# rajashree-srikanth/drone-sim-python

Hardware: AMD Instinct MI355X
Metric: trajectory-optimisations/sec (6-seg poly, 50 wpts) (higher is better)
Workload: dtype f64 residual/gradient + f32 MFMA J^T J

## Files before the change

### drone-sim-python_amd/csrc/asan_host.cpp

```cpp
#include <cmath>
#include <cstdarg>
#include <cstdio>
#include <string>

#include "fit_plan.h"

static std::string g_err;
void d2d_set_error(const char *fmt, ...) {
  char buf[512];
  va_list ap;
  va_start(ap, fmt);
  vsnprintf(buf, sizeof(buf), fmt, ap);
  va_end(ap);
  g_err = buf;
}

static int check_plan(int S, int K, double duration) {
  d2d_fit_plan pl;
  pl.device = 0; pl.S = S; pl.K = K; pl.duration = duration;
  const double s = 0.1 / K;
  pl.wref[0] = 4e-4; pl.wref[1] = 5.0 * s; pl.wref[2] = s / (9.81 * 9.81);
  const int rc = fit_basis_build(&pl);
  if (rc != 0) { std::printf("S=%d K=%d: rc=%d (%s)\n", S, K, rc, g_err.c_str()); return rc; }
  const int nq = pl.nq;
  double worst = 0.0;
  for (int i = 0; i < nq; ++i)
    for (int j = 0; j < nq; ++j) {
      double acc = 0.0;
      for (int k = 0; k < K; ++k) acc += pl.Pinit[(size_t)i * K + k] * pl.G[(size_t)k * nq + j];
      worst = std::fmax(worst, std::fabs(acc - (i == j ? 1.0 : 0.0)));
    }
  std::printf("S=%d K=%d nq=%d: |Pinit G0 - I| = %.2e\n", S, K, nq, worst);
  if (int rc2 = fit_basis_segments(&pl)) { std::printf("  segments: rc=%d (%s)\n", rc2, g_err.c_str()); return rc2; }
  double wseg = 0.0, gmax = 0.0;
  const double c1 = 2.0 / pl.T;
  for (int k = 0; k < K; ++k) {
    const double x = pl.sx[k];
    double P[8], d1[8], d2[8];
    P[0] = 1; P[1] = x; d1[0] = 0; d1[1] = 1; d2[0] = d2[1] = 0;
    for (int n = 1; n < 7; ++n) {
      P[n + 1] = ((2.0 * n + 1.0) * x * P[n] - n * P[n - 1]) / (n + 1.0);
      d1[n + 1] = d1[n - 1] + (2.0 * n + 1.0) * P[n];
      d2[n + 1] = d2[n - 1] + (2.0 * n + 1.0) * d1[n];
    }
    for (int d = 0; d < 3; ++d)
      for (int j = 0; j < nq; ++j) {
        double acc = 0.0;
        for (int i = 0; i < 8; ++i) {
          const double psi = d == 0 ? P[i] : (d == 1 ? c1 * d1[i] : c1 * c1 * d2[i]);
          acc += psi * pl.Zl[(size_t)(8 * pl.seg[k] + i) * nq + j];
        }
        const double gv = pl.G[((size_t)d * K + k) * nq + j];
        wseg = std::fmax(wseg, std::fabs(acc - gv));
        gmax = std::fmax(gmax, std::fabs(gv));
      }
  }
  int lanes = 0, covered = 0, zlbig = 0;
  for (int s = 0; s < S; ++s) {
    const int L = pl.seg_l0[s + 1] - pl.seg_l0[s];
    lanes += L;
    covered += pl.seg_Ks[s];
    if (L < 1 || (pl.seg_Ks[s] + L - 1) / L > pl.seg_nchunk) zlbig = 1;
  }
  double zlmax = 0.0;
  for (double v : pl.Zl) zlmax = std::fmax(zlmax, std::fabs(v));
  std::printf("  segments: |Psi Zl - G| = %.2e of %.2e, |Zl| <= %.2f, %d lanes, %d chunks\n", wseg, gmax, zlmax, lanes, pl.seg_nchunk);
  if (!(wseg < 1e-9 * gmax) || lanes > 64 || covered != K || zlbig || !(zlmax < 50.0)) return 1;
  return worst < 1e-6 ? 0 : 1;
}

int main() {
  int bad = 0;
  const int shapes[][2] = {{6, 50}, {6, 61}, {6, 121}, {6, 151}, {6, 501}, {3, 20}, {1, 8}, {4, 31}};
  for (auto &sh : shapes) bad += check_plan(sh[0], sh[1], 0.1 * (sh[1] - 1)) != 0;
  d2d_fit_plan pl;
  pl.device = 0; pl.S = 6; pl.K = 18; pl.duration = 1.0; pl.wref[0] = 4e-4; pl.wref[1] = 1e-2; pl.wref[2] = 1e-5;
  const int rc = fit_basis_build(&pl);
  std::printf("S=6 K=18 (rank-deficient): rc=%d (%s)\n", rc, g_err.c_str());
  bad += rc == 0;
  std::printf(bad ? "asan_host: FAILED\n" : "asan_host: ok\n");
  return bad;
}
```

### drone-sim-python_amd/csrc/fit_basis.cpp

```cpp
#include <cmath>
#include <cstring>

#include "fit_plan.h"

namespace {

double arr(int k, int n) {
  double a = 1;
  for (int i = n; i > n - k; --i) a *= i;
  return a;
}

struct Dense {
  int r, c;
  std::vector<double> a;
  Dense(int r_, int c_) : r(r_), c(c_), a((size_t)r_ * c_, 0.0) {}
  double &operator()(int i, int j) { return a[(size_t)i * c + j]; }
  double operator()(int i, int j) const { return a[(size_t)i * c + j]; }
};

Dense matmul(const Dense &A, const Dense &B, bool tA = false) {
  const int m = tA ? A.c : A.r, k = tA ? A.r : A.c, n = B.c;
  Dense C(m, n);
  for (int i = 0; i < m; ++i)
    for (int l = 0; l < k; ++l) {
      const double v = tA ? A(l, i) : A(i, l);
      if (v == 0.0) continue;
      for (int j = 0; j < n; ++j) C(i, j) += v * B(l, j);
    }
  return C;
}

bool cholesky(Dense &A) {
  const int n = A.r;
  for (int j = 0; j < n; ++j) {
    double d = A(j, j);
    for (int k = 0; k < j; ++k) d -= A(j, k) * A(j, k);
    if (!(d > 0.0)) return false;
    d = std::sqrt(d);
    A(j, j) = d;
    for (int i = j + 1; i < n; ++i) {
      double s = A(i, j);
      for (int k = 0; k < j; ++k) s -= A(i, k) * A(j, k);
      A(i, j) = s / d;
    }
    for (int i = 0; i < j; ++i) A(i, j) = 0.0;
  }
  return true;
}

bool invert(Dense &A) {
  const int n = A.r;
  Dense I(n, n);
// ... 229 lines not shown
          (best < 0 || chunks(s) > chunks(best) || (chunks(s) == chunks(best) && pl->seg_Ks[s] * L[best] > pl->seg_Ks[best] * L[s])))
        best = s;
    if (best < 0) break;
    L[best]++;
  }
  pl->seg_nchunk = 0;
  pl->seg_l0[0] = 0;
  for (int s = 0; s < S; ++s) {
    pl->seg_l0[s + 1] = pl->seg_l0[s] + L[s];
    if (chunks(s) > pl->seg_nchunk) pl->seg_nchunk = chunks(s);
  }
  for (int s = S; s < D2D_FIT_MAX_S; ++s) pl->seg_l0[s + 1] = pl->seg_l0[S];
  return D2D_OK;
}

int fit_basis_knots(d2d_fit_plan *pl) {
  const int S = pl->S, K = pl->K, nq = pl->nq, NE = 8 * (S + 1);
  const double T = pl->T;
  if (nq != 4 * S || (int)pl->Lw.size() != nq * nq) { d2d_set_error("fit_basis_knots: plan without the whitening factor"); return D2D_EINVAL; }
  auto &kn = pl->kn;
  kn.NE = NE;
  double dsc[4] = {1.0, T, T * T / 2.0, T * T * T / 6.0};
  std::vector<int> freec;
  for (int i = 0; i < 4 * (S + 1); ++i)
    if (i != 0 && i != 1 && i != 4 * S && i != 4 * S + 1) freec.push_back(i);
  const int NV = 4 * (S + 1);
  kn.NV = NV;
  std::vector<int> vfree(NV, -1);
  for (int i = 0; i < nq; ++i) vfree[freec[i]] = i;
  Dense A(8, 8);
  for (int k = 0; k < 4; ++k) {
    A(k, k) = 1.0;
    for (int p = k; p < 8; ++p) {
      double c = 1.0;
      for (int i = 0; i < k; ++i) c = c * (p - i) / (i + 1);
      A(4 + k, p) = c;
    }
  }
  if (!invert(A)) { d2d_set_error("fit_basis_knots: singular Hermite block"); return D2D_EINVAL; }
  kn.Hb64.assign((size_t)K * KN_HB_STRIDE, 0.0);
  kn.Hb32.assign((size_t)K * 32, 0.f);
  for (int k = 0; k < K; ++k) {
    const double x = pl->tau[k] / T;
    const int s = pl->seg[k];
    for (int d = 0; d < 3; ++d)
      for (int m = 0; m < 8; ++m) {
        double v = 0.0;
        for (int p = d; p < 8; ++p) v += arr(d, p) * std::pow(x, p - d) * A(p, m);
        v /= std::pow(T, d);
        kn.Hb64[(size_t)k * KN_HB_STRIDE + 4 * m + d] = v;
        const bool fixed = (s == 0 && m < 2) || (s == S - 1 && m >= 4 && m < 6);
        kn.Hb32[(size_t)k * 32 + 4 * m + d] = fixed ? 0.f : (float)v;
      }
  }
  fit_knot_first_samples(pl->seg, S, kn.k0);
  kn.Wseg.assign((size_t)S * 4 * 64, 0.f);
  for (int s = 0; s < S; ++s)
    for (int r = 0; r < 4; ++r)
      for (int l = 0; l < 64; ++l) {
        const int R = 4 * (l >> 4) + r, C = l & 15;
        const int aR = (R >> 2) & 1, aC = (C >> 2) & 1, mR = 4 * (R >> 3) + (R & 3), mC = 4 * (C >> 3) + (C & 3);
        if (aR != aC) continue;
        double v = 0.0;
        for (int k = kn.k0[s]; k < kn.k0[s + 1]; ++k) v += (double)kn.Hb32[(size_t)k * 32 + 4 * mR] * (double)kn.Hb32[(size_t)k * 32 + 4 * mC];
        kn.Wseg[((size_t)s * 4 + r) * 64 + l] = (float)v;
      }
  Dense L(nq, nq), Bm(nq, nq), Bi(nq, nq), Mu(nq, nq);
  for (int i = 0; i < nq; ++i)
    for (int j = 0; j < nq; ++j) L(i, j) = pl->Lw[(size_t)i * nq + j];
  std::vector<double> ds(nq);
  for (int i = 0; i < nq; ++i) ds[i] = dsc[freec[i] % 4];
  for (int j = 0; j < nq; ++j)
    for (int i = 0; i < nq; ++i) Bm(j, i) = L(i, j) / ds[i];
  Bi = Bm;
  if (!invert(Bi)) { d2d_set_error("fit_basis_knots: singular map"); return D2D_EINVAL; }
  Mu = matmul(Bm, Bm, true);
  Dense Mi = Mu;
  if (!invert(Mi)) { d2d_set_error("fit_basis_knots: singular metric"); return D2D_EINVAL; }
  kn.Bq.assign((size_t)2 * nq * NV, 0.0);
  kn.BiT.assign((size_t)2 * nq * NV, 0.0);
  kn.Md32.assign((size_t)2 * nq * 2 * nq, 0.f);
  kn.Mrow32.assign((size_t)NE * 12, 0.f);
  kn.Binv.assign((size_t)NE * nq, 0.0);
  kn.Minv.assign((size_t)NE * NV, 0.0);
  kn.Mrow.assign((size_t)NE * 12, 0.0);
  kn.Pu.assign((size_t)NE * 4, 0.0);
  kn.msc.assign((size_t)NE, 1.0);
  for (int a = 0; a < 2; ++a)
    for (int jq = 0; jq < nq; ++jq)
      for (int i = 0; i < nq; ++i) {
        kn.Bq[((size_t)a * nq + jq) * NV + freec[i]] = Bm(jq, i);
        kn.BiT[((size_t)a * nq + jq) * NV + freec[i]] = Bi(i, jq);
      }
  for (int e = 0; e < NE; ++e) {
    const int j = e >> 3, k = e & 3, v = 4 * j + k, i = vfree[v];
    if (i < 0) {
      kn.Pu[(size_t)e * 4 + (j == 0 ? k : 2 + k)] = dsc[k];
      continue;
    }
    for (int c = 0; c < 4; ++c) kn.Pu[(size_t)e * 4 + c] = ds[i] * pl->Pe[(size_t)i * 4 + c];
    for (int jq = 0; jq < nq; ++jq) kn.Binv[(size_t)e * nq + jq] = Bi(i, jq);
    for (int i2 = 0; i2 < nq; ++i2) kn.Minv[(size_t)e * NV + freec[i2]] = Mi(i, i2);
    for (int dj = -1; dj <= 1; ++dj)
      for (int k2 = 0; k2 < 4; ++k2) {
        const int v2 = 4 * (j + dj) + k2;
        if (v2 < 0 || v2 >= NV || vfree[v2] < 0) continue;
// ... 24 lines not shown
```

### drone-sim-python_amd/csrc/fit_knot.hip

```cpp
#include <cstdlib>
#include <vector>

#include "fit_phases.h"
#include "fit_plan.h"

#define KN_WPB_MAX 8
#define KN_LDS_BYTES (160 * 1024)
#define KN_N 48
#define KN_NE 56
#define KN_WV_KNOT 10
#define KN_US 10
#define KN_GTOL_SCALE 0.1
#define KN_SEG_MAX 11
#define KN_FUSED_DEPTH 6
#define KN_SEG_FLOOR 8
#define KN_IMG_LS (KN_N + 4)

namespace {

#define LAUNDER_S(v) do { (v) = __builtin_amdgcn_readfirstlane(v); asm volatile("" : "+s"(v)); } while (0)

struct KnotGeom {
  int K, S, smax;
  int k0[D2D_FIT_MAX_S + 2];
// ... 126 lines not shown
          h01[i] = *reinterpret_cast<const f64x2a *>(hb + i * KN_HB_STRIDE); u01[i] = *reinterpret_cast<const f64x2a *>(uk + i * KN_US);
          h2[i] = hb[i * KN_HB_STRIDE + 2]; u2[i] = uk[i * KN_US + 2];
        } else {
          h01[i] = f64x2a{0.0, 0.0}; u01[i] = f64x2a{0.0, 0.0}; h2[i] = 0.0; u2[i] = 0.0;
        }
#pragma unroll
      for (int i = 0; i < 3; ++i) {
        a0 = fma(h01[i].x, u01[i].x, a0);
        a1 = fma(h01[i].y, u01[i].y, a1);
        a2 = fma(h2[i], u2[i], a2);
      }
      hb += 3 * KN_HB_STRIDE; uk += 3 * KN_US;
    }
  }
  return (a0 + a1) + a2;
}

template <int SEGMAX>
__device__ __forceinline__ void knot_mfma(const KnotGeom &kg, const unsigned char *lds, int hb32_off, int cf_off, const float *Wseg,
                                          float ww, int lane, f32x4 (&acc)[D2D_FIT_MAX_S]) {
  LAUNDER(lane);
  const int c = lane & 15, r = lane >> 4;
  const int m = 4 * (c >> 3) + (c & 3), a = (c >> 2) & 1;
  const int tab = hb32_off + (4 * m + (r < 2 ? 1 : 0)) * 4;
  const int cfo = cf_off + r * 16 + a * 8;
#pragma unroll
  for (int s0 = 0; s0 < D2D_FIT_MAX_S; s0 += 3) {
    float v[3][SEGMAX];
    int n[3];
#pragma unroll
    for (int j = 0; j < 3; ++j) {
      const int s = s0 + j;
      int kb = kg.k0[s];
      n[j] = kg.k0[s + 1] - kg.k0[s];
      LAUNDER_S(kb); LAUNDER_S(n[j]);
#pragma unroll
      for (int i = 0; i < SEGMAX; ++i) {
        const int kk = kb + (i < n[j] ? i : (n[j] > 0 ? n[j] - 1 : 0));
        const float2 t = lds_get<float2>(lds + tab + kk * 128);
        const float2 cc = lds_get<float2>(lds + cfo + kk * 64);
        v[j][i] = fmaf(cc.y, t.y, cc.x * t.x);
      }
#pragma unroll
      for (int rr = 0; rr < 4; ++rr) acc[s][rr] = ww * Wseg[(s * 4 + rr) * 64 + lane];
    }
#pragma unroll
    for (int i = 0; i < SEGMAX; ++i)
#pragma unroll
      for (int j = 0; j < 3; ++j)
        if (i < n[j]) acc[s0 + j] = __builtin_amdgcn_mfma_f32_16x16x4f32(v[j][i], v[j][i], acc[s0 + j], 0, 0, 0);
  }
}

template <int SEGMAX, int SEGMIN>
__device__ __forceinline__ double knot_eval_fused(const KnotGeom &kg, const unsigned char *lds, const double *Hb64, const double *us,
                                                  int kb, int km, int ke, int a, int kd, bool live, int hb32_off, int cf_off,
                                                  const float *Wseg, float ww, int lane, f32x4 (&acc)[D2D_FIT_MAX_S]) {
  typedef double __attribute__((ext_vector_type(2), may_alias)) f64x2a;
  constexpr int SLOTS = (SEGMAX + 2) / 3 * 3;
  static_assert(SEGMIN > 0 && SEGMIN <= SEGMAX && SEGMIN % 3 != 0, "a masked sample follows the floor in every half");
  static_assert(D2D_FIT_MAX_S == 6, "two halves of three segments");
  LAUNDER(lane);
  LAUNDER(kb);
  const int c = lane & 15, r = lane >> 4;
  const int m = 4 * (c >> 3) + (c & 3), ax = (c >> 2) & 1;
  const int tab = hb32_off + (4 * m + (r < 2 ? 1 : 0)) * 4;
  const int cfo = cf_off + r * 16 + ax * 8;
  double a0 = 0.0, a1 = 0.0, a2 = 0.0;
#pragma unroll
  for (int half = 0; half < 2; ++half) {
    const int s0 = 3 * half;
    const int k0 = half ? km : kb, k1 = half ? ke : km;
    const int n = live ? k1 - k0 : 0;
    const bool some = n > 0;
    const int k0r = some ? k0 : 0;
    const double *hb = Hb64 + (size_t)k0r * KN_HB_STRIDE + 4 * ((half ? 0 : 4) + kd);
    const double *uk = us + k0r * KN_US + 4 * a;
    const double b0 = a0, b1 = a1, b2 = a2;
    constexpr int NQ = 3 * SEGMIN, TAIL = SEGMAX - SEGMIN, DEPTH = KN_FUSED_DEPTH;
    static_assert(SEGMIN >= 4, "the operand pipeline is two rows deep");
    const unsigned char *tp[3], *cp[3];
    float2 rt[DEPTH], rc[DEPTH], rtt[3][TAIL > 0 ? TAIL : 1], rct[3][TAIL > 0 ? TAIL : 1];
    float vq[2], vt[3][TAIL > 0 ? TAIL : 1];
    int ns[3];
#pragma unroll
    for (int j = 0; j < 3; ++j) {
      const int s = s0 + j;
      int sb = kg.k0[s];
      ns[j] = kg.k0[s + 1] - kg.k0[s];
      LAUNDER_S(sb); LAUNDER_S(ns[j]);
      tp[j] = lds + tab + sb * 128; cp[j] = lds + cfo + sb * 64;
#pragma unroll
      for (int i = 0; i < DEPTH / 3; ++i) { rt[3 * i + j] = lds_get<float2>(tp[j] + i * 128); rc[3 * i + j] = lds_get<float2>(cp[j] + i * 64); }
#pragma unroll
      for (int rr = 0; rr < 4; ++rr) acc[s][rr] = ww * Wseg[(s * 4 + rr) * 64 + lane];
    }
    vq[0] = fmaf(rc[0].y, rt[0].y, rc[0].x * rt[0].x);
    __builtin_amdgcn_sched_barrier(0);
    constexpr int LAG = 3, STEP = (NQ - 1 - LAG) / (SLOTS - 1), NBUF = LAG / (STEP > 0 ? STEP : 1) + 1;
    static_assert(STEP >= 1, "every sample of the half finds its two k-steps");
    f64x2a h01[NBUF], u01[NBUF];
    double h2[NBUF], u2[NBUF];
    auto p2_read = [&](int idx, int i) {
      if (idx < SEGMIN) {
        h01[i] = *reinterpret_cast<const f64x2a *>(hb + idx * KN_HB_STRIDE); u01[i] = *reinterpret_cast<const f64x2a *>(uk + idx * KN_US);
        h2[i] = hb[idx * KN_HB_STRIDE + 2]; u2[i] = uk[idx * KN_US + 2];
      } else {
        const bool in = idx < n;
        const int o = in ? idx : 0;
        const f64x2a hr = *reinterpret_cast<const f64x2a *>(hb + o * KN_HB_STRIDE), ur = *reinterpret_cast<const f64x2a *>(uk + o * KN_US);
        const double h2r = hb[o * KN_HB_STRIDE + 2], u2r = uk[o * KN_US + 2];
        h01[i] = in ? hr : f64x2a{0.0, 0.0}; u01[i] = in ? ur : f64x2a{0.0, 0.0};
        h2[i] = in ? h2r : 0.0; u2[i] = in ? u2r : 0.0;
      }
    };
    auto p2_fma = [&](int idx, int i) {
      if (idx == SEGMIN) { a0 = some ? a0 : b0; a1 = some ? a1 : b1; a2 = some ? a2 : b2; }
      a0 = fma(h01[i].x, u01[i].x, a0);
      a1 = fma(h01[i].y, u01[i].y, a1);
      a2 = fma(h2[i], u2[i], a2);
      LAUNDER(a0); LAUNDER(a1); LAUNDER(a2);
    };
#pragma unroll
    for (int q = 0; q < NQ; ++q) {
      const int i = q / 3, j = q % 3;
      acc[s0 + j] = __builtin_amdgcn_mfma_f32_16x16x4f32(vq[q & 1], vq[q & 1], acc[s0 + j], 0, 0, 0);
      if (q + DEPTH < NQ) {
        rt[q % DEPTH] = lds_get<float2>(tp[j] + (i + DEPTH / 3) * 128); rc[q % DEPTH] = lds_get<float2>(cp[j] + (i + DEPTH / 3) * 64);
      } else if (q + 6 < NQ + 3 && q + 6 >= NQ) {
#pragma unroll
        for (int t = 0; t < TAIL; ++t) {
          const int kk = SEGMIN + t < ns[j] ? SEGMIN + t : ns[j] - 1;
          rtt[j][t] = lds_get<float2>(tp[j] + kk * 128); rct[j][t] = lds_get<float2>(cp[j] + kk * 64);
        }
      } else if (q + 3 >= NQ) {
#pragma unroll
        for (int t = 0; t < TAIL; ++t) vt[j][t] = fmaf(rct[j][t].y, rtt[j][t].y, rct[j][t].x * rtt[j][t].x);
      }
      if (q % STEP == 0 && q / STEP < SLOTS) p2_read(q / STEP, (q / STEP) % NBUF);
      if (q >= LAG && (q - LAG) % STEP == 0 && (q - LAG) / STEP < SLOTS) p2_fma((q - LAG) / STEP, ((q - LAG) / STEP) % NBUF);
      if (q + 1 < NQ) vq[(q + 1) & 1] = fmaf(rc[(q + 1) % DEPTH].y, rt[(q + 1) % DEPTH].y, rc[(q + 1) % DEPTH].x * rt[(q + 1) % DEPTH].x);
      __builtin_amdgcn_sched_barrier(0);
    }
#pragma unroll
    for (int t = 0; t < TAIL; ++t)
#pragma unroll
      for (int j = 0; j < 3; ++j)
        if (SEGMIN + t < ns[j]) acc[s0 + j] = __builtin_amdgcn_mfma_f32_16x16x4f32(vt[j][t], vt[j][t], acc[s0 + j], 0, 0, 0);
  }
  return (a0 + a1) + a2;
}

__device__ __forceinline__ void knot_mfma_so(const KnotGeom &kg, const unsigned char *lds, int hb32_off, int cf_off, int cfp_off,
                                             const float *Wseg, float ww, int lane, f32x4 (&acc)[D2D_FIT_MAX_S]) {
  LAUNDER(lane);
  const int c = lane & 15, rho = lane >> 4;
  const int m = 4 * (c >> 3) + (c & 3);
  const bool ay = ((c >> 2) & 1) != 0, row_y = (rho & 1) != 0, row_2 = rho >= 2;
  const int tab = hb32_off + 4 * m * 4;
  const int reco = cf_off + rho * 16 + (ay ? 8 : 0), rpo = cfp_off + (rho & 1) * 8 + (ay ? 4 : 0);
#pragma unroll
  for (int s = 0; s < D2D_FIT_MAX_S; ++s) {
#pragma unroll
    for (int rr = 0; rr < 4; ++rr) acc[s][rr] = ww * Wseg[(s * 4 + rr) * 64 + lane];
    int k1 = kg.k0[s + 1];
    int k = kg.k0[s];
    LAUNDER_S(k1); LAUNDER_S(k);
    if (k < k1) {
      f32x4 hb = lds_get<f32x4>(lds + tab + k * 128);
      float2 rec = lds_get<float2>(lds + reco + k * 64);
      float rp = lds_get<float>(lds + rpo + k * 16);
      for (; k < k1; ++k) {
        const int kn = k + 1 < k1 ? k + 1 : k;
        const f32x4 hbn = lds_get<f32x4>(lds + tab + kn * 128);
        const float2 recn = lds_get<float2>(lds + reco + kn * 64);
        const float rpn = lds_get<float>(lds + rpo + kn * 16);
        const float h0 = hb.x, h1 = hb.y, h2 = hb.z;
        const float cx = rec.x, cy = rec.y;
        const float vb = fmaf(cy, h2, cx * h1);
        const float va = (row_y == ay) ? (row_2 ? h2 : h1) : 0.f;
        acc[s] = __builtin_amdgcn_mfma_f32_16x16x4f32(va, vb, acc[s], 0, 0, 0);
        const float vbp = row_2 ? 0.f : rp * h0;
        const float vap = (!row_2 && row_y == ay) ? h0 : 0.f;
        acc[s] = __builtin_amdgcn_mfma_f32_16x16x4f32(vap, vbp, acc[s], 0, 0, 0);
        hb = hbn; rec = recn; rp = rpn;
      }
    }
  }
}

__device__ __forceinline__ void knot_blocks_to_image(f32x4 (&acc)[D2D_FIT_MAX_S], float *Hs, int lane) {
  LAUNDER(lane);
  constexpr int LS = KN_IMG_LS;
  for (int i = lane; i < KN_N * LS / 4; i += 64) lds_put<f32x4>(Hs + 4 * i, f32x4{0.f, 0.f, 0.f, 0.f});
  const int c = lane & 15, g4 = lane >> 4;
  const bool lowq = c < 8 && g4 < 2, highq = c >= 8 && g4 >= 2;
  const int src = ((lane + 40) & 63) << 2;
  auto fetch = [&](float v) -> float {
    const float up = __builtin_bit_cast(float, __builtin_amdgcn_ds_bpermute(src, __builtin_bit_cast(int, v)));
    return lowq ? up : 0.f;
  };
#pragma unroll
  for (int s = D2D_FIT_MAX_S - 1; s >= 1; --s) {
    const float u0 = fetch(acc[s - 1].x), u1 = fetch(acc[s - 1].y), u2 = fetch(acc[s - 1].z), u3 = fetch(acc[s - 1].w);
    acc[s].x += u0; acc[s].y += u1; acc[s].z += u2; acc[s].w += u3;
  }
  wave_lds_sync();
  const int cq = c & 7, cd = 2 * (cq >> 2) + (cq & 3) - 2;
  const bool cv = (cq & 3) >= 2;
#pragma unroll
  for (int s = 0; s < D2D_FIT_MAX_S; ++s) {
    int iC = 8 * s + c - 4;
    bool okc = true;
    if (s == 0) { iC = c < 8 ? cd : c - 4; okc = c >= 8 || cv; }
    if (s == D2D_FIT_MAX_S - 1) { iC = c < 8 ? 8 * s + c - 4 : 44 + cd; okc = c < 8 || cv; }
    const bool mine = okc && !(highq && s < D2D_FIT_MAX_S - 1);
#pragma unroll
    for (int rr = 0; rr < 4; ++rr) {
      int iR = 8 * s + 4 * g4 + rr - 4;
      bool okr = true;
      if (s == 0 && rr < 2) okr = g4 >= 2;
      if (s == 0 && rr >= 2) iR = g4 < 2 ? 2 * g4 + rr - 2 : 4 * g4 + rr - 4;
      if (s == D2D_FIT_MAX_S - 1 && rr < 2) okr = g4 < 2;
      if (s == D2D_FIT_MAX_S - 1 && rr >= 2) iR = g4 < 2 ? 8 * s + 4 * g4 + rr - 4 : 44 + 2 * (g4 - 2) + rr - 2;
      if (mine && okr) Hs[iR * LS + iC] = acc[s][rr];
    }
  }
  wave_lds_sync();
}

struct KnotMetric {
  unsigned char *lds;
  int sfull_off, md32_off, mr32_off;
  int lane;
  float lam;
  float scale;
  __device__ __forceinline__ float apply(float v) const {
#ifdef KN_ABL_APPLY
    return v;
#endif
    int l = lane;
    LAUNDER(l);
    const bool act = l < KN_N;
    const int e = act ? kn_entry_of(l) : 0;
    float *sf = reinterpret_cast<float *>(lds + sfull_off);
    wave_lds_sync();
    if (act) sf[8 + e] = v;
    wave_lds_sync();
    const float *bq = sf + 8 * (e >> 3) + 4 * ((e >> 2) & 1);
    const float *mrow = reinterpret_cast<const float *>(lds + mr32_off) + e * 12;
    const f32x4 s0 = lds_get<f32x4>(bq), s1 = lds_get<f32x4>(bq + 8), s2 = lds_get<f32x4>(bq + 16);
    const f32x4 m0 = lds_get<f32x4>(mrow), m1 = lds_get<f32x4>(mrow + 4), m2 = lds_get<f32x4>(mrow + 8);
    float r = m0.x * s0.x;
    r = fmaf(m0.y, s0.y, r); r = fmaf(m0.z, s0.z, r); r = fmaf(m0.w, s0.w, r);
    r = fmaf(m1.x, s1.x, r); r = fmaf(m1.y, s1.y, r); r = fmaf(m1.z, s1.z, r); r = fmaf(m1.w, s1.w, r);
    r = fmaf(m2.x, s2.x, r); r = fmaf(m2.y, s2.y, r); r = fmaf(m2.z, s2.z, r); r = fmaf(m2.w, s2.w, r);
    return act ? r : 0.f;
  }
  int row_off;
  __device__ __forceinline__ void prepare(int l) { row_off = md32_off + ((l < KN_N && lam != 0.f) ? l : KN_N) * (KN_N * 4); }
  __device__ __forceinline__ f32x4 damp(int j0) const {
#ifdef KN_ABL_DAMP
    return f32x4{lam, lam, lam, lam};
#endif
    return lds_get<f32x4>(reinterpret_cast<const float *>(lds + row_off) + j0);
  }
};

}
template <> struct nd_is_banded<KnotMetric> { static constexpr bool value = true; };
static_assert(KN_N == 48 && D2D_FIT_MAX_S == 6, "nd_panel3_chunk0_zero<KnotMetric> rests on the 4 / 8 x 5 / 4 layout of the 48 free entries");
template <> struct nd_panel3_chunk0_zero<KnotMetric> { static constexpr bool value = true; };
namespace {

template <bool STAMPS, bool SEG9, int SEGMIN>
__global__ void __launch_bounds__(64 * KN_WPB_MAX)
fit_lm_knot_kernel(int B, KnotGeom kg, KnotLds L, d2d_fit_opts opts, int iter_cap, KnotDev T, const double *__restrict__ pk,
                   const double *__restrict__ prep, double *q_io, double *cost_io, double *g_io, double *lm, int32_t *flags,
                   int32_t *queue, const int32_t *__restrict__ order, int prio_at, double *u_io, unsigned long long *__restrict__ stamps,
                   float *dbg) {
  unsigned long long st_acc[8] = {0, 0, 0, 0, 0, 0, 0, 0}, st_last = 0;
#define KN_STAMP(i)                                                     \
  if (STAMPS) {                                                         \
    const unsigned long long t_ = __builtin_amdgcn_s_memtime();         \
    st_acc[i] += t_ - st_last;                                          \
    st_last = t_;                                                       \
  }
  extern __shared__ __attribute__((aligned(16))) unsigned char lds[];
  constexpr int N = KN_N;
  stage(lds + L.Hb64, T.Hb64, kg.K * KN_HB_STRIDE * 8);
  stage(lds + L.Hb32, T.Hb32, kg.K * 32 * 4);
  stage(lds + L.Wseg, T.Wseg, D2D_FIT_MAX_S * 4 * 64 * 4);
  stage(lds + L.Md32, T.Md32, N * N * 4);
  stage(lds + L.Mi32, T.Mi32, KN_NE * 28 * 4);
  stage(lds + L.Mr32, T.Mrow32, KN_NE * 12 * 4);
  stage(lds + L.Msc, T.msc, KN_NE * 8);
  for (int i = threadIdx.x; i < N; i += blockDim.x) reinterpret_cast<float *>(lds + L.Md32)[N * N + i] = 0.f;
  __syncthreads();
  const double *Hb64 = reinterpret_cast<const double *>(lds + L.Hb64);
  const float *Wseg = reinterpret_cast<const float *>(lds + L.Wseg);
  const float *Mi32 = reinterpret_cast<const float *>(lds + L.Mi32);
  const int wave = __builtin_amdgcn_readfirstlane(threadIdx.x >> 6), lane = threadIdx.x & 63;
  unsigned char *wl = lds + L.wave0 + wave * L.wave_stride;
  double *wv = reinterpret_cast<double *>(wl + L.wv);
  double *sp = reinterpret_cast<double *>(wl + L.sp);
  float *sfull = reinterpret_cast<float *>(wl + L.sfull);
  double *gfull = reinterpret_cast<double *>(wl + L.gfull);
  double *park = reinterpret_cast<double *>(wl + L.park);
  double *us = reinterpret_cast<double *>(wl + L.big);
  f32x4 *cf = reinterpret_cast<f32x4 *>(wl + L.cf);
  float2 *cfp = reinterpret_cast<float2 *>(wl + L.cfp);
  float *big = reinterpret_cast<float *>(wl + L.big);
  const bool act = lane < N;
  const int e = kn_entry_all(lane);
  const int ej = e >> 3, ea = (e >> 2) & 1, ekd = e & 3;
  const int wv_slot = ej * KN_WV_KNOT + 4 * ea + ekd;
  auto p2_ranges = [&](int &kb, int &km, int &ke) {
    int lj = lane;
    LAUNDER(lj);
    const int e2 = lj < N ? kn_entry_of(lj) : 0, j2 = e2 >> 3;
    kb = 0; km = 0; ke = 0;
#pragma unroll
    for (int j = 0; j <= D2D_FIT_MAX_S; ++j)
      if (j == j2) { kb = kg.k0[j > 0 ? j - 1 : 0]; km = kg.k0[j]; ke = kg.k0[j < kg.S ? j + 1 : kg.S]; }
  };
  auto seg_of_lane = [&]() -> int {
    int lj = lane;
    LAUNDER(lj);
    int sg = 0;
#pragma unroll
    for (int s = 1; s < D2D_FIT_MAX_S; ++s) sg += (lj >= kg.k0[s] && s < kg.S) ? 1 : 0;
    return sg;
  };
  auto msc_of_lane = [&]() -> double {
    int l = lane;
    LAUNDER(l);
    return reinterpret_cast<const double *>(lds + L.Msc)[l < N ? kn_entry_of(l) : 0];
  };
  for (int i = lane; i < 9 * 8; i += 64) sfull[i] = 0.f;
  KnotMetric metric;
  metric.lds = lds; metric.sfull_off = L.wave0 + wave * L.wave_stride + L.sfull; metric.md32_off = L.Md32; metric.mr32_off = L.Mr32;
  metric.lane = lane; metric.lam = 0.f; metric.scale = 0.f; metric.row_off = 0;
// ... 81 lines not shown
#define V_qmax u2
#define V_ct u3
#define V_pred_s u4
#define V_bt_a u5
#define V_bt_b u6
#define V_alpha u7
    int nev = 0, status = D2D_ST_RUNNING;
    bool so_rows = uniform_i(lmb[3] != 0.0 ? 1 : 0) != 0;
    int phase = 1;
    MpState mp;
    mp.pgn_lds = nullptr;
    mp.dx_gn = 0.0; mp.t2_gn = 0.0; mp.p_gn = 0.f; mp.gn_valid = 0; mp.gn_ok = 0; mp.first = 0; mp.calm = 0; mp.slow = 0; mp.nfac = 0;
    {
      const int pw = uniform_i((int)lmb[6]);
      phase = pw & 1; mp.first = (pw >> 1) & 1; mp.calm = (pw >> 2) & 0x3fff; mp.slow = pw >> 16;
    }
    if (phase == 0) { V_mp_par = uniform_d(lmb[4]); V_mp_delta = uniform_d(lmb[5]); }
    else { V_lam = uniform_d(lmb[0]); V_nu = uniform_d(lmb[1]); }
    double c = 0.0, gi = 0.0, gnrm = -1.0, xub = 0.0;
    float hdiag = 0.f;
    f32x2 hrow[N / 2];
#pragma unroll
    for (int m = 0; m < N / 2; ++m) hrow[m] = f32x2{0.f, 0.f};
    wave_lds_sync();
    if (phase == 0) {
      const float dv = act ? (float)(ui - u0_of_lane()) : 0.f;
      const float mv = metric.apply(dv);
      const double xn = sqrt(fmax(uniform_d(wave_sum((double)dv * (double)mv)), 0.0));
      xub = xn * (1.0 + 1e-6);
      if (mp.first && V_mp_delta <= 0.0) V_mp_delta = xn > 0.0 ? 100.0 * xn : 100.0;
    }
    KN_STAMP(0)
    for (bool reenter = true; reenter;) {
      reenter = false;
      c = uniform_d(knot_phase1(kg.K, Hb64, sp, wv, seg_of_lane(), park, us, cf, cfp, so_rows, lane));
      KN_STAMP(1)
      bool fresh = true;
      if (!(fabs(c) <= 1.79e308)) { status = D2D_ST_NONFINITE; fresh = false; }
      int sub = 0, lp_it = 0, att = 0;
      V_alpha = 1.0;
      float dl = 0.f;
      bool fin = false, accept = false;
      while (status == D2D_ST_RUNNING || fresh) {
        bool do_solve = false, is_gn = false, do_trial = false;
        double solve_lam = 0.0;
        int isq_mode = 0;
        if (sub == 0) {
          if (fresh) {
            int p2_kb, p2_km, p2_ke;
            p2_ranges(p2_kb, p2_km, p2_ke);
            f32x4 acc[D2D_FIT_MAX_S];
            const float ww = (float)(sp[PR_WWP] * sp[PR_WWP]);
            const int wbase = L.wave0 + wave * L.wave_stride;
            const bool fused = SEGMIN > 0 && !so_rows && status == D2D_ST_RUNNING;
            if (!fused) gi = knot_phase2(kg, Hb64, us, p2_kb, p2_km, p2_ke, ea, ekd, act, lane);
            KN_STAMP(2)
            fresh = false;
            if (status != D2D_ST_RUNNING) break;
            if (so_rows) knot_mfma_so(kg, lds, L.Hb32, wbase + L.cf, wbase + L.cfp, Wseg, ww, lane, acc);
            else if constexpr (SEGMIN > 0)
              gi = knot_eval_fused<(SEG9 ? 9 : KN_SEG_MAX), SEGMIN>(kg, lds, Hb64, us, p2_kb, p2_km, p2_ke, ea, ekd, act, L.Hb32, wbase + L.cf,
                                                                    Wseg, ww, lane, acc);
            else if (SEG9) knot_mfma<9>(kg, lds, L.Hb32, wbase + L.cf, Wseg, ww, lane, acc);
            else knot_mfma<KN_SEG_MAX>(kg, lds, L.Hb32, wbase + L.cf, Wseg, ww, lane, acc);
            nev += so_rows ? 3 : 2;
            wave_lds_sync();
            KN_STAMP(3)
            knot_blocks_to_image(acc, big, lane);
            image_put_rhs<N>(big, lane, gi);
            wave_lds_sync();
            image_row<N>(big, lane, hrow);
            hdiag = image_diag<N>(big, lane);
            wave_lds_sync();
            if (STAMPS && dbg != nullptr && iters == 0 && act) {
              float *d = dbg + (size_t)b * (N * N + 4 * N) + lane * N;
#pragma unroll
              for (int m = 0; m < N / 2; ++m) { d[2 * m] = hrow[m].x; d[2 * m + 1] = hrow[m].y; }
              dbg[(size_t)b * (N * N + 4 * N) + N * N + lane] = (float)gi;
              dbg[(size_t)b * (N * N + 4 * N) + N * N + N + lane] = (float)ui;
            }
            gnrm = -1.0;
            KN_STAMP(4)
          }
          if (iters >= iter_cap || iters >= opts.max_iter) break;
          if (iters >= prio_at) __builtin_amdgcn_s_setprio(2);
          if (phase == 0) {
            const double fnorm = sqrt(c);
            double gl = 0.0;
            if (act && hdiag > 0.f && fnorm > 0.0) gl = fabs(gi) / (sqrt((double)hdiag) * fnorm);
            V_gnorm = uniform_d(wave_max(gl));
            if (V_gnorm <= opts.mp_gtol) { status = D2D_ST_CONVERGED; break; }
            V_par = V_mp_par; V_parl = 0.0; V_paru = 0.0; V_fp = 0.0; lp_it = 0; V_alpha = 1.0;
            if (!mp.gn_valid) { do_solve = true; is_gn = true; solve_lam = 0.0; isq_mode = 1; }
            else sub = 3;
          } else {
            const double gmax = uniform_d(wave_max(act ? fabs(gi) / msc_of_lane() : 0.0));
            if (gmax <= KN_GTOL_SCALE * opts.gtol) { status = D2D_ST_CONVERGED; break; }
            do_solve = true; solve_lam = V_lam;
          }
        } else if (sub == 1) {
          if (V_par == 0.0) V_par = fmax(MP_DWARF, 0.001 * V_paru);
          do_solve = true; solve_lam = V_par; isq_mode = lp_it + 1 < 10 ? 2 : 0;
        } else if (sub == 2) {
          do_trial = true;
        }
        bool ok = true;
        if (do_solve) {
          double dxn = 0.0, t2 = 0.0;
          float dls, dgi;
          metric.lam = lane < N ? (float)solve_lam : 0.f; metric.scale = metric.lam;
          ok = uniform_i(damped_solve<N, true, true>(hrow, 0.0, act, lane, big, dgi, dls, nullptr, true, isq_mode, V_mp_delta, &dxn, &t2,
                                                     hdiag, true, metric) ? 1 : 0) != 0;
          KN_STAMP(5)
// ... 377 lines not shown
```

Before: 1.815 million.

## Add software-pipelined second-order MFMA path with fused phase-2 gradient rider

Pulls the fp64 phase-2 gradient accumulation out into a reusable rider struct and adds a new knot_mfma_so_floor kernel for the second-order-rows path. The new kernel pipelines LDS operand loads one row ahead of the MFMA issue, handles tail samples separately, and, when SEG9 is set, folds the phase-2 dot product into the same loop instead of running knot_phase2 on its own. A host-side check that the fp32 Hermite table's pad words are +0.f is added, since the new kernel loads three-word vectors that can touch the pad word. The cost is more code paths and higher register pressure from the extra tail buffers.

Measured after the change: 1.897 million, median of 6. 1.05x the previous value.

```diff
diff --git a/drone-sim-python_amd/csrc/asan_host.cpp b/drone-sim-python_amd/csrc/asan_host.cpp
--- a/drone-sim-python_amd/csrc/asan_host.cpp
+++ b/drone-sim-python_amd/csrc/asan_host.cpp
@@ -1,6 +1,8 @@
 #include <cmath>
 #include <cstdarg>
+#include <cstdint>
 #include <cstdio>
+#include <cstring>
 #include <string>
 
 #include "fit_plan.h"
@@ -66,12 +68,24 @@
   for (double v : pl.Zl) zlmax = std::fmax(zlmax, std::fabs(v));
   std::printf("  segments: |Psi Zl - G| = %.2e of %.2e, |Zl| <= %.2f, %d lanes, %d chunks\n", wseg, gmax, zlmax, lanes, pl.seg_nchunk);
   if (!(wseg < 1e-9 * gmax) || lanes > 64 || covered != K || zlbig || !(zlmax < 50.0)) return 1;
+  if (S == 6 && nq == 24 && K <= 64) {
+    if (int rc3 = fit_basis_knots(&pl)) { std::printf("  knots: rc=%d (%s)\n", rc3, g_err.c_str()); return rc3; }
+    int pads = 0, filled = 0;
+    for (size_t i = 0; i < pl.kn.Hb32.size(); ++i) {
+      uint32_t bits;
+      std::memcpy(&bits, &pl.kn.Hb32[i], sizeof(bits));
+      if (i % 4 == 3) pads += bits != 0u;
+      else filled += bits != 0u;
+    }
+    std::printf("  knots: fp32 Hermite table of %zu words, %d filled, %d pad words not +0.f\n", pl.kn.Hb32.size(), filled, pads);
+    if ((int)pl.kn.Hb32.size() != K * 32 || pads != 0 || filled == 0) return 1;
+  }
   return worst < 1e-6 ? 0 : 1;
 }
 
 int main() {
   int bad = 0;
-  const int shapes[][2] = {{6, 50}, {6, 61}, {6, 121}, {6, 151}, {6, 501}, {3, 20}, {1, 8}, {4, 31}};
+  const int shapes[][2] = {{6, 50}, {6, 48}, {6, 64}, {6, 61}, {6, 121}, {6, 151}, {6, 501}, {3, 20}, {1, 8}, {4, 31}};
   for (auto &sh : shapes) bad += check_plan(sh[0], sh[1], 0.1 * (sh[1] - 1)) != 0;
   d2d_fit_plan pl;
   pl.device = 0; pl.S = 6; pl.K = 18; pl.duration = 1.0; pl.wref[0] = 4e-4; pl.wref[1] = 1e-2; pl.wref[2] = 1e-5;
diff --git a/drone-sim-python_amd/csrc/fit_basis.cpp b/drone-sim-python_amd/csrc/fit_basis.cpp
--- a/drone-sim-python_amd/csrc/fit_basis.cpp
+++ b/drone-sim-python_amd/csrc/fit_basis.cpp
@@ -1,4 +1,5 @@
 #include <cmath>
+#include <cstdint>
 #include <cstring>
 
 #include "fit_plan.h"
@@ -334,6 +335,11 @@
         const bool fixed = (s == 0 && m < 2) || (s == S - 1 && m >= 4 && m < 6);
         kn.Hb32[(size_t)k * 32 + 4 * m + d] = fixed ? 0.f : (float)v;
       }
+  }
+  for (size_t i = 3; i < kn.Hb32.size(); i += 4) {
+    uint32_t bits;
+    std::memcpy(&bits, &kn.Hb32[i], sizeof(bits));
+    if (bits != 0u) { d2d_set_error("fit_basis_knots: pad word %zu of the fp32 Hermite table is not +0.f", i); return D2D_EINVAL; }
   }
   fit_knot_first_samples(pl->seg, S, kn.k0);
   kn.Wseg.assign((size_t)S * 4 * 64, 0.f);
diff --git a/drone-sim-python_amd/csrc/fit_knot.hip b/drone-sim-python_amd/csrc/fit_knot.hip
--- a/drone-sim-python_amd/csrc/fit_knot.hip
+++ b/drone-sim-python_amd/csrc/fit_knot.hip
@@ -202,13 +202,59 @@
   }
 }
 
+template <int SEGMAX, int SEGMIN, int NQ>
+struct KnotP2Rider {
+  typedef double __attribute__((ext_vector_type(2), may_alias)) f64x2a;
+  static constexpr int SLOTS = (SEGMAX + 2) / 3 * 3;
+  static constexpr int LAG = 3, STEP = (NQ - 1 - LAG) / (SLOTS - 1), NBUF = LAG / (STEP > 0 ? STEP : 1) + 1;
+  static_assert(SEGMIN > 0 && SEGMIN <= SEGMAX && SEGMIN % 3 != 0, "a masked sample follows the floor in every half");
+  static_assert(STEP >= 1, "every sample of the half finds its two k-steps");
+  const double *hb, *uk;
+  int n;
+  bool some;
+  double a0 = 0.0, a1 = 0.0, a2 = 0.0, b0, b1, b2;
+  f64x2a h01[NBUF], u01[NBUF];
+  double h2[NBUF], u2[NBUF];
+  __device__ __forceinline__ void begin(int half, const double *Hb64, const double *us, int kb, int km, int ke, int a, int kd, bool live) {
+    const int k0 = half ? km : kb, k1 = half ? ke : km;
+    n = live ? k1 - k0 : 0;
+    some = n > 0;
+    const int k0r = some ? k0 : 0;
+    hb = Hb64 + (size_t)k0r * KN_HB_STRIDE + 4 * ((half ? 0 : 4) + kd);
+    uk = us + k0r * KN_US + 4 * a;
+    b0 = a0; b1 = a1; b2 = a2;
+  }
+  __device__ __forceinline__ void read(int idx, int i) {
+    if (idx < SEGMIN) {
+      h01[i] = *reinterpret_cast<const f64x2a *>(hb + idx * KN_HB_STRIDE); u01[i] = *reinterpret_cast<const f64x2a *>(uk + idx * KN_US);
+      h2[i] = hb[idx * KN_HB_STRIDE + 2]; u2[i] = uk[idx * KN_US + 2];
+    } else {
+      const bool in = idx < n;
+      const int o = in ? idx : 0;
+      const f64x2a hr = *reinterpret_cast<const f64x2a *>(hb + o * KN_HB_STRIDE), ur = *reinterpret_cast<const f64x2a *>(uk + o * KN_US);
+      const double h2r = hb[o * KN_HB_STRIDE + 2], u2r = uk[o * KN_US + 2];
+      h01[i] = in ? hr : f64x2a{0.0, 0.0}; u01[i] = in ? ur : f64x2a{0.0, 0.0};
+      h2[i] = in ? h2r : 0.0; u2[i] = in ? u2r : 0.0;
+    }
+  }
+  __device__ __forceinline__ void fma3(int idx, int i) {
+    if (idx == SEGMIN) { a0 = some ? a0 : b0; a1 = some ? a1 : b1; a2 = some ? a2 : b2; }
+    a0 = fma(h01[i].x, u01[i].x, a0);
+    a1 = fma(h01[i].y, u01[i].y, a1);
+    a2 = fma(h2[i], u2[i], a2);
+    LAUNDER(a0); LAUNDER(a1); LAUNDER(a2);
+  }
+  __device__ __forceinline__ void step(int q) {
+    if (q % STEP == 0 && q / STEP < SLOTS) read(q / STEP, (q / STEP) % NBUF);
+    if (q >= LAG && (q - LAG) % STEP == 0 && (q - LAG) / STEP < SLOTS) fma3((q - LAG) / STEP, ((q - LAG) / STEP) % NBUF);
+  }
+  __device__ __forceinline__ double sum() const { return (a0 + a1) + a2; }
+};
+
 template <int SEGMAX, int SEGMIN>
 __device__ __forceinline__ double knot_eval_fused(const KnotGeom &kg, const unsigned char *lds, const double *Hb64, const double *us,
                                                   int kb, int km, int ke, int a, int kd, bool live, int hb32_off, int cf_off,
                                                   const float *Wseg, float ww, int lane, f32x4 (&acc)[D2D_FIT_MAX_S]) {
-  typedef double __attribute__((ext_vector_type(2), may_alias)) f64x2a;
-  constexpr int SLOTS = (SEGMAX + 2) / 3 * 3;
-  static_assert(SEGMIN > 0 && SEGMIN <= SEGMAX && SEGMIN % 3 != 0, "a masked sample follows the floor in every half");
   static_assert(D2D_FIT_MAX_S == 6, "two halves of three segments");
   LAUNDER(lane);
   LAUNDER(kb);
@@ -216,17 +262,11 @@
   const int m = 4 * (c >> 3) + (c & 3), ax = (c >> 2) & 1;
   const int tab = hb32_off + (4 * m + (r < 2 ? 1 : 0)) * 4;
   const int cfo = cf_off + r * 16 + ax * 8;
-  double a0 = 0.0, a1 = 0.0, a2 = 0.0;
+  KnotP2Rider<SEGMAX, SEGMIN, 3 * SEGMIN> p2;
 #pragma unroll
   for (int half = 0; half < 2; ++half) {
     const int s0 = 3 * half;
-    const int k0 = half ? km : kb, k1 = half ? ke : km;
-    const int n = live ? k1 - k0 : 0;
-    const bool some = n > 0;
-    const int k0r = some ? k0 : 0;
-    const double *hb = Hb64 + (size_t)k0r * KN_HB_STRIDE + 4 * ((half ? 0 : 4) + kd);
-    const double *uk = us + k0r * KN_US + 4 * a;
-    const double b0 = a0, b1 = a1, b2 = a2;
+    p2.begin(half, Hb64, us, kb, km, ke, a, kd, live);
     constexpr int NQ = 3 * SEGMIN, TAIL = SEGMAX - SEGMIN, DEPTH = KN_FUSED_DEPTH;
     static_assert(SEGMIN >= 4, "the operand pipeline is two rows deep");
     const unsigned char *tp[3], *cp[3];
@@ -247,30 +287,6 @@
     }
     vq[0] = fmaf(rc[0].y, rt[0].y, rc[0].x * rt[0].x);
     __builtin_amdgcn_sched_barrier(0);
-    constexpr int LAG = 3, STEP = (NQ - 1 - LAG) / (SLOTS - 1), NBUF = LAG / (STEP > 0 ? STEP : 1) + 1;
-    static_assert(STEP >= 1, "every sample of the half finds its two k-steps");
-    f64x2a h01[NBUF], u01[NBUF];
-    double h2[NBUF], u2[NBUF];
-    auto p2_read = [&](int idx, int i) {
-      if (idx < SEGMIN) {
-        h01[i] = *reinterpret_cast<const f64x2a *>(hb + idx * KN_HB_STRIDE); u01[i] = *reinterpret_cast<const f64x2a *>(uk + idx * KN_US);
-        h2[i] = hb[idx * KN_HB_STRIDE + 2]; u2[i] = uk[idx * KN_US + 2];
-      } else {
-        const bool in = idx < n;
-        const int o = in ? idx : 0;
-        const f64x2a hr = *reinterpret_cast<const f64x2a *>(hb + o * KN_HB_STRIDE), ur = *reinterpret_cast<const f64x2a *>(uk + o * KN_US);
-        const double h2r = hb[o * KN_HB_STRIDE + 2], u2r = uk[o * KN_US + 2];
-        h01[i] = in ? hr : f64x2a{0.0, 0.0}; u01[i] = in ? ur : f64x2a{0.0, 0.0};
-        h2[i] = in ? h2r : 0.0; u2[i] = in ? u2r : 0.0;
-      }
-    };
-    auto p2_fma = [&](int idx, int i) {
-      if (idx == SEGMIN) { a0 = some ? a0 : b0; a1 = some ? a1 : b1; a2 = some ? a2 : b2; }
-      a0 = fma(h01[i].x, u01[i].x, a0);
-      a1 = fma(h01[i].y, u01[i].y, a1);
-      a2 = fma(h2[i], u2[i], a2);
-      LAUNDER(a0); LAUNDER(a1); LAUNDER(a2);
-    };
 #pragma unroll
     for (int q = 0; q < NQ; ++q) {
       const int i = q / 3, j = q % 3;
@@ -287,8 +303,7 @@
 #pragma unroll
         for (int t = 0; t < TAIL; ++t) vt[j][t] = fmaf(rct[j][t].y, rtt[j][t].y, rct[j][t].x * rtt[j][t].x);
       }
-      if (q % STEP == 0 && q / STEP < SLOTS) p2_read(q / STEP, (q / STEP) % NBUF);
-      if (q >= LAG && (q - LAG) % STEP == 0 && (q - LAG) / STEP < SLOTS) p2_fma((q - LAG) / STEP, ((q - LAG) / STEP) % NBUF);
+      p2.step(q);
       if (q + 1 < NQ) vq[(q + 1) & 1] = fmaf(rc[(q + 1) % DEPTH].y, rt[(q + 1) % DEPTH].y, rc[(q + 1) % DEPTH].x * rt[(q + 1) % DEPTH].x);
       __builtin_amdgcn_sched_barrier(0);
     }
@@ -298,7 +313,7 @@
       for (int j = 0; j < 3; ++j)
         if (SEGMIN + t < ns[j]) acc[s0 + j] = __builtin_amdgcn_mfma_f32_16x16x4f32(vt[j][t], vt[j][t], acc[s0 + j], 0, 0, 0);
   }
-  return (a0 + a1) + a2;
+  return p2.sum();
 }
 
 __device__ __forceinline__ void knot_mfma_so(const KnotGeom &kg, const unsigned char *lds, int hb32_off, int cf_off, int cfp_off,
@@ -337,6 +352,97 @@
       }
     }
   }
+}
+
+template <int SEGMAX, int SEGMIN, bool RIDER>
+__device__ __forceinline__ double knot_mfma_so_floor(const KnotGeom &kg, const unsigned char *lds, const double *Hb64, const double *us,
+                                                     int kb, int km, int ke, int a, int kd, bool live, int hb32_off, int cf_off,
+                                                     int cfp_off, const float *Wseg, float ww, int lane, f32x4 (&acc)[D2D_FIT_MAX_S]) {
+  static_assert(SEGMIN >= 2 && SEGMIN <= SEGMAX, "the operand pipeline is one row of k-steps deep");
+  static_assert(D2D_FIT_MAX_S == 6 && KN_FUSED_DEPTH == 6, "two halves of three segments; a k-step's words are fetched one row of the half ahead");
+  typedef float __attribute__((ext_vector_type(3))) f32x3;
+  LAUNDER(lane);
+  LAUNDER(kb);
+  const int c = lane & 15, rho = lane >> 4;
+  const int m = 4 * (c >> 3) + (c & 3);
+  const bool ay = ((c >> 2) & 1) != 0, row_y = (rho & 1) != 0, row_2 = rho >= 2;
+  const bool own = row_y == ay;
+  const int tab = hb32_off + 4 * m * 4;
+  const int tab_a = tab + (own ? (row_2 ? 8 : 4) : 12), tab_p = tab + (own && !row_2 ? 0 : 12);
+  const int reco = cf_off + rho * 16 + (ay ? 8 : 0), rpo = cfp_off + (rho & 1) * 8 + (ay ? 4 : 0);
+  constexpr int NQ = 6 * SEGMIN, TAIL = SEGMAX - SEGMIN, NT = TAIL > 0 ? TAIL : 1;
+  KnotP2Rider<SEGMAX, SEGMIN, NQ> p2;
+#pragma unroll
+  for (int half = 0; half < 2; ++half) {
+    const int s0 = 3 * half;
+    if constexpr (RIDER) p2.begin(half, Hb64, us, kb, km, ke, a, kd, live);
+    const unsigned char *th[3], *ta[3], *tp[3], *cp[3], *pp[3];
+    f32x3 rh[3];
+    float2 rc[3];
+    float ra[3], rh0[3], rp[3], rap[3];
+    f32x3 rht[3][NT];
+    float2 rct[3][NT];
+    float rat[3][NT], rpt[3][NT], rapt[3][NT];
+    float va[2], vb[2], vat[3][NT], vbt[3][NT], vapt[3][NT], vbpt[3][NT];
+    int ns[3];
+#pragma unroll
+    for (int j = 0; j < 3; ++j) {
+      const int s = s0 + j;
+      int sb = kg.k0[s];
+      ns[j] = kg.k0[s + 1] - kg.k0[s];
+      LAUNDER_S(sb); LAUNDER_S(ns[j]);
+      th[j] = lds + tab + sb * 128; ta[j] = lds + tab_a + sb * 128; tp[j] = lds + tab_p + sb * 128;
+      cp[j] = lds + reco + sb * 64; pp[j] = lds + rpo + sb * 16;
+      rh[j] = lds_get<f32x3>(th[j]); rc[j] = lds_get<float2>(cp[j]); ra[j] = lds_get<float>(ta[j]);
+#pragma unroll
+      for (int rr = 0; rr < 4; ++rr) acc[s][rr] = ww * Wseg[(s * 4 + rr) * 64 + lane];
+    }
+#pragma unroll
+    for (int j = 0; j < 3; ++j) { rp[j] = lds_get<float>(pp[j]); rap[j] = lds_get<float>(tp[j]); }
+    va[0] = ra[0]; vb[0] = fmaf(rc[0].y, rh[0].z, rc[0].x * rh[0].y); rh0[0] = rh[0].x;
+    __builtin_amdgcn_sched_barrier(0);
+    auto form = [&](int q) {
+      const int t = (q / 3) & 1, j = q % 3;
+      if (t == 0) { va[q & 1] = ra[j]; vb[q & 1] = fmaf(rc[j].y, rh[j].z, rc[j].x * rh[j].y); rh0[j] = rh[j].x; }
+      else { va[q & 1] = rap[j]; vb[q & 1] = row_2 ? 0.f : rp[j] * rh0[j]; }
+    };
+#pragma unroll
+    for (int q = 0; q < NQ; ++q) {
+      const int i = q / 6, t = (q / 3) & 1, j = q % 3;
+      acc[s0 + j] = __builtin_amdgcn_mfma_f32_16x16x4f32(va[q & 1], vb[q & 1], acc[s0 + j], 0, 0, 0);
+      if (q + 6 < NQ) {
+        if (t == 0) { rh[j] = lds_get<f32x3>(th[j] + (i + 1) * 128); rc[j] = lds_get<float2>(cp[j] + (i + 1) * 64); ra[j] = lds_get<float>(ta[j] + (i + 1) * 128); }
+        else { rp[j] = lds_get<float>(pp[j] + (i + 1) * 16); rap[j] = lds_get<float>(tp[j] + (i + 1) * 128); }
+      } else {
+#pragma unroll
+        for (int tt = 0; tt < TAIL; ++tt) {
+          const int kk = SEGMIN + tt < ns[j] ? SEGMIN + tt : ns[j] - 1;
+          if (t == 0) { rht[j][tt] = lds_get<f32x3>(th[j] + kk * 128); rct[j][tt] = lds_get<float2>(cp[j] + kk * 64); rat[j][tt] = lds_get<float>(ta[j] + kk * 128); }
+          else { rpt[j][tt] = lds_get<float>(pp[j] + kk * 16); rapt[j][tt] = lds_get<float>(tp[j] + kk * 128); }
+        }
+        if (t == 1) {
+#pragma unroll
+          for (int tt = 0; tt < TAIL; ++tt) { vat[j][tt] = rat[j][tt]; vbt[j][tt] = fmaf(rct[j][tt].y, rht[j][tt].z, rct[j][tt].x * rht[j][tt].y); }
+        }
+      }
+      if constexpr (RIDER) p2.step(q);
+      if (q + 1 < NQ) form(q + 1);
+      __builtin_amdgcn_sched_barrier(0);
+    }
+#pragma unroll
+    for (int tt = 0; tt < TAIL; ++tt)
+#pragma unroll
+      for (int j = 0; j < 3; ++j) { vapt[j][tt] = rapt[j][tt]; vbpt[j][tt] = row_2 ? 0.f : rpt[j][tt] * rht[j][tt].x; }
+#pragma unroll
+    for (int tt = 0; tt < TAIL; ++tt)
+#pragma unroll
+      for (int j = 0; j < 3; ++j)
+        if (SEGMIN + tt < ns[j]) {
+          acc[s0 + j] = __builtin_amdgcn_mfma_f32_16x16x4f32(vat[j][tt], vbt[j][tt], acc[s0 + j], 0, 0, 0);
+          acc[s0 + j] = __builtin_amdgcn_mfma_f32_16x16x4f32(vapt[j][tt], vbpt[j][tt], acc[s0 + j], 0, 0, 0);
+        }
+  }
+  return RIDER ? p2.sum() : 0.0;
 }
 
 __device__ __forceinline__ void knot_blocks_to_image(f32x4 (&acc)[D2D_FIT_MAX_S], float *Hs, int lane) {
@@ -438,6 +544,7 @@
   }
   extern __shared__ __attribute__((aligned(16))) unsigned char lds[];
   constexpr int N = KN_N;
+  constexpr bool SO_RIDER = SEGMIN > 0 && SEG9;
   stage(lds + L.Hb64, T.Hb64, kg.K * KN_HB_STRIDE * 8);
   stage(lds + L.Hb32, T.Hb32, kg.K * 32 * 4);
   stage(lds + L.Wseg, T.Wseg, D2D_FIT_MAX_S * 4 * 64 * 4);
@@ -625,13 +732,18 @@
             f32x4 acc[D2D_FIT_MAX_S];
             const float ww = (float)(sp[PR_WWP] * sp[PR_WWP]);
             const int wbase = L.wave0 + wave * L.wave_stride;
-            const bool fused = SEGMIN > 0 && !so_rows && status == D2D_ST_RUNNING;
+            const bool fused = SEGMIN > 0 && (!so_rows || SO_RIDER) && status == D2D_ST_RUNNING;
             if (!fused) gi = knot_phase2(kg, Hb64, us, p2_kb, p2_km, p2_ke, ea, ekd, act, lane);
             KN_STAMP(2)
             fresh = false;
             if (status != D2D_ST_RUNNING) break;
-            if (so_rows) knot_mfma_so(kg, lds, L.Hb32, wbase + L.cf, wbase + L.cfp, Wseg, ww, lane, acc);
-            else if constexpr (SEGMIN > 0)
+            if (so_rows) {
+              if constexpr (SEGMIN > 0) {
+                const double g2 = knot_mfma_so_floor<(SEG9 ? 9 : KN_SEG_MAX), SEGMIN, SO_RIDER>(kg, lds, Hb64, us, p2_kb, p2_km, p2_ke, ea, ekd, act, L.Hb32,
+                                                                                                  wbase + L.cf, wbase + L.cfp, Wseg, ww, lane, acc);
+                if (SO_RIDER) gi = g2;
+              } else knot_mfma_so(kg, lds, L.Hb32, wbase + L.cf, wbase + L.cfp, Wseg, ww, lane, acc);
+            } else if constexpr (SEGMIN > 0)
               gi = knot_eval_fused<(SEG9 ? 9 : KN_SEG_MAX), SEGMIN>(kg, lds, Hb64, us, p2_kb, p2_km, p2_ke, ea, ekd, act, L.Hb32, wbase + L.cf,
                                                                     Wseg, ww, lane, acc);
             else if (SEG9) knot_mfma<9>(kg, lds, L.Hb32, wbase + L.cf, Wseg, ww, lane, acc);
```
